# JuliaGenAI/ColBERT.jl

Measured on AMD Instinct MI355X. Metric: queries/sec, top-1000 on 1M-passage corpus, higher is better.
Workload: dtype f32

## Files before the change

### colbert.jl_amd/csrc/approx_kernels.hpp

```cpp
#pragma once
#include <hip/hip_fp16.h>

#include <algorithm>

#include "common.hpp"
#include "search_kernels.hpp"

namespace clb {

typedef __bf16 bf16x8 __attribute__((ext_vector_type(8)));
typedef uint32_t u32x4 __attribute__((ext_vector_type(4)));
typedef uint32_t u32x4_a4 __attribute__((ext_vector_type(4), aligned(4)));
typedef float f32x4_a4 __attribute__((ext_vector_type(4), aligned(4)));

constexpr float kEpsSafety = 1.25f;

inline bool approx_supported(int dim, int nbits) { return dim == kDim && nbits == 2; }
inline size_t approx_cells_bytes(int64_t B, int64_t K, int64_t ) { return (size_t)B * K * 16 * 4 + 2048; }

__device__ __forceinline__ uint32_t f32_to_bf16_rne(float f) {
    const uint32_t u = __float_as_uint(f);
    return (u + 0x7fffu + ((u >> 16) & 1u)) >> 16;
}
__device__ __forceinline__ uint32_t pack_bf16(float lo, float hi) {
// ... 860 lines not shown
    const uint32_t cmask = (1u << cbits) - 1u;
    const int lane = threadIdx.x & 63;
    const int r = lane & 31, h = lane >> 5;
    const int x = blockIdx.x & 7;
    const int wg = blockIdx.x >> 3;
    const int wg_per_group = gridDim.x >> 3;
    const int wave = __builtin_amdgcn_readfirstlane(threadIdx.x >> 6);
    __shared__ __attribute__((aligned(16))) unsigned char lut_s[kApproxLdsLut];
    __shared__ __attribute__((aligned(16))) float invx[kApproxThreads / 64][2 * kStepRows];
    constexpr int kSlotBytes = CELL8 ? 1024 : 2048;
    constexpr int kRingBytes = 3 * kSlotBytes;
    __shared__ __attribute__((aligned(16))) unsigned char ring_s[GL ? (kApproxThreads / 64) * kRingBytes : 16];
    constexpr int kStageBytes = 16 * 64 + 64;
    __shared__ __attribute__((aligned(16))) unsigned char stage_s[ROWS ? 16 : (kApproxThreads / 64) * kStageBytes];
    unsigned char* mystage = stage_s + (ROWS ? 0 : wave * kStageBytes);
    for (int i = threadIdx.x; i < 256 * 32; i += kApproxThreads) {
        const int v = i >> 5;
        *reinterpret_cast<uint2*>(lut_s + (size_t)i * 8) =
            make_uint2(pack_f16(weights[v & 3], weights[(v >> 2) & 3]), pack_f16(weights[(v >> 4) & 3], weights[(v >> 6) & 3]));
    }
    __syncthreads();
    const char* lut = reinterpret_cast<const char*>(lut_s);
    float* myinv = invx[wave];
    const uint32_t lane8 = 8u * (uint32_t)r;
    unsigned char* myring = ring_s + (GL ? wave * kRingBytes : 0);
    const uint32_t ring_lds = (uint32_t)(uintptr_t)(__attribute__((address_space(3))) unsigned char*)myring;
    const uint32_t gl_poff = 16u * (((uint32_t)lane - (((uint32_t)lane >> 4) & 3u)) & 3u);
    const int gl_src0 = (int)((uint32_t)lane & ~3u);
    const int gl_src1 = gl_src0 + 64;
    const uint32_t gl_rot = ((uint32_t)r >> 2) & 3u;
// ... 31 lines not shown
                float4 hi = *reinterpret_cast<const float4*>(qrow + 8 * s + 4);
                if (r >= T) { lo = make_float4(0.f, 0.f, 0.f, 0.f); hi = lo; }
                if (CELL8) {
                    lo.x *= ts.y; lo.y *= ts.y; lo.z *= ts.y; lo.w *= ts.y;
                    hi.x *= ts.y; hi.y *= ts.y; hi.z *= ts.y; hi.w *= ts.y;
                }
                qb[s] = u32x4{pack_f16(lo.x, lo.y), pack_f16(lo.z, lo.w), pack_f16(hi.x, hi.y), pack_f16(hi.z, hi.w)};
            }
        }
        const uint2* hdr = cand_hdr + (size_t)b * cand_cap;
        const char* c16 = reinterpret_cast<const char*>(cells16 + (size_t)b * K * (CELL8 ? 8 : 16));
        const uint32_t h16 = 16u * (uint32_t)h;
        float* out = scores + (size_t)b * cand_cap;
        uint16_t* tmax = tokmax + (size_t)b * cand_cap * 32 + r;
        const int* lst = ROWS ? list + (size_t)b * cand_cap : nullptr;
        unsigned long long* rmask = ROWS ? rowmask + (size_t)b * cand_cap * 4 : nullptr;
        const float window = ROWS ? 2.f * eps_pair[b] : 0.f;
        const int n = ROWS ? nlist[b] : ncand[b];
        const int n_waves = wg_count * (kApproxThreads / 64) * nsub;
        const int my_wave = (sub * wg_count + wg_index) * (kApproxThreads / 64) + wave;
        const int per_wave = (n + n_waves - 1) / n_waves;
        const int j_first = min(n, my_wave * per_wave), j_end = min(n, j_first + per_wave);
        unsigned long long wm0 = 0, wm1 = 0, wm2 = 0, wm3 = 0;

        for (int j0 = j_first; j0 < j_end; j0 += 64) {
        const int jl = j0 + lane;
        int slot_l = jl < j_end ? jl : j0;
        if (ROWS) slot_l = lst[slot_l];
        const uint2 hv = hdr[slot_l];
        const int nd = j_end - j0 < 64 ? j_end - j0 : 64;
        int it_k = 0;
        uint32_t it_off = __builtin_amdgcn_readlane(hv.x, 0);
        int it_len = (int)__builtin_amdgcn_readlane(hv.y, 0);
        int it_slot = __builtin_amdgcn_readlane(slot_l, 0);
        int it_base = 0;

#define CLB_STAGE_A(RB, CV, PM, TAG)                                                                    \
    {                                                                                                       \
// ... 147 lines not shown
         \
        float v[16];                                                                                        \
        _Pragma("unroll") for (int i = 0; i < 16; ++i) { v[i] = ACC[i] * iq[i >> 2][i & 3]; asm volatile("" : "+v"(v[i])); } \
        if (ROWS) {                                                                                         \
            const __half pmh = *reinterpret_cast<const __half*>(&PM);                                       \
            const float lo = r < T ? __half2float(pmh) - window : __builtin_inff();    \
             \
             \
             \
            uint32_t lm = 0;                                                                                \
            _Pragma("unroll") for (int i = 0; i < 16; ++i) lm |= !((CELL8 ? v[i] * stp : v[i]) < lo) ? (1u << i) : 0u; \
            lm |= (uint32_t)__builtin_amdgcn_update_dpp(0, (int)lm, 0xB1, 0xf, 0xf, true);         \
            lm |= (uint32_t)__builtin_amdgcn_update_dpp(0, (int)lm, 0x4E, 0xf, 0xf, true);         \
            lm |= (uint32_t)__builtin_amdgcn_update_dpp(0, (int)lm, 0x141, 0xf, 0xf, true);    \
            lm |= (uint32_t)__builtin_amdgcn_update_dpp(0, (int)lm, 0x140, 0xf, 0xf, true);      \
            const uint32_t m0_ = __builtin_amdgcn_readlane(lm, 0) | __builtin_amdgcn_readlane(lm, 16);      \
            const uint32_t m1_ = __builtin_amdgcn_readlane(lm, 32) | __builtin_amdgcn_readlane(lm, 48);     \
             \
            uint32_t bits = ((m0_ & 0xFu) | ((m0_ & 0xF0u) << 4) | ((m0_ & 0xF00u) << 8) | ((m0_ & 0xF000u) << 12)) | \
                            (((m1_ & 0xFu) | ((m1_ & 0xF0u) << 4) | ((m1_ & 0xF00u) << 8) | ((m1_ & 0xF000u) << 12)) << 4); \
            if (TAG.rows < kStepRows) bits &= (1u << TAG.rows) - 1u;        \
            const unsigned long long wbits = (unsigned long long)bits << (TAG.base & 32);                   \
            const int wi = TAG.base >> 6;                                                                   \
            wm0 |= wi == 0 ? wbits : 0ull;                                                                  \
            wm1 |= wi == 1 ? wbits : 0ull;                                                                  \
            wm2 |= wi == 2 ? wbits : 0ull;                                                                  \
            wm3 |= wi == 3 ? wbits : 0ull;                                                                  \
            if (TAG.last) {                                                                                 \
                if (lane == 0 && TAG.j >= 0) {                                                              \
                    unsigned long long* o = rmask + (size_t)TAG.j * 4;                                      \
                    o[0] = wm0; o[1] = wm1; o[2] = wm2; o[3] = wm3;                                         \
                }                                                                                           \
                wm0 = wm1 = wm2 = wm3 = 0;                                                                  \
            }                                                                                               \
        } else {                                                                                            \
            if (TAG.g) {               \
                const float q0_ = fmaxf(fmaxf(fmaxf(v[0], v[1]), v[2]), v[3]);                              \
                const float q1_ = fmaxf(fmaxf(fmaxf(v[4], v[5]), v[6]), v[7]);                              \
                const float q2_ = fmaxf(fmaxf(fmaxf(v[8], v[9]), v[10]), v[11]);                            \
                const float q3_ = fmaxf(fmaxf(fmaxf(v[12], v[13]), v[14]), v[15]);                          \
                const float mh_ = fmaxf(fmaxf(mx, q0_), fmaxf(TAG.g > 1 ? q1_ : kNegInf, TAG.g > 2 ? q2_ : kNegInf)); \
                CLB_PASSAGE_END(mh_, TAG.jh, 1);                                                            \
                mx = fmaxf(fmaxf(TAG.g > 1 ? kNegInf : q1_, TAG.g > 2 ? kNegInf : q2_), q3_);               \
            } else {                                                                                        \
            float m01 = fmaxf(fmaxf(v[0], v[1]), v[2]);                                                     \
            float m23 = fmaxf(fmaxf(v[3], v[4]), v[5]);                                                     \
            float m45 = fmaxf(fmaxf(v[6], v[7]), v[8]);                                                     \
            float m67 = fmaxf(fmaxf(v[9], v[10]), v[11]);                                                   \
// ... 589 lines not shown
```

### colbert.jl_amd/csrc/search.hip

```cpp
#include <algorithm>
#include <atomic>
#include <cstdlib>
#include <cstring>
#include <memory>
#include <numeric>

#include "append_kernels.hpp"
#include "approx_kernels.hpp"
#include "generic_kernels.hpp"
#include "remove_kernels.hpp"
#include "search_kernels.hpp"
#include "sort.hpp"

using namespace clb;

namespace {

enum KernelId {
    KID_CENTROID_SCORES = 0,
    KID_TOPN,
    KID_MARK,
    KID_COMPACT,
    KID_SCORE_EXACT,
    KID_SCORE_APPROX,
// ... 209 lines not shown
    }
    CLB_TRY(w.cand_hdr.ensure(sizeof(uint2) * B * w.cand_cap));
    CLB_TRY(w.scores.ensure(sizeof(float) * B * w.cand_cap));
    CLB_TRY(w.list.ensure(sizeof(int) * B * w.cand_cap));
    CLB_TRY(w.nlist.ensure(sizeof(int) * B));
    CLB_TRY(w.thresh.ensure(sizeof(float) * B * 2));
    CLB_TRY(w.outp.ensure(sizeof(int64_t) * B * k));
    CLB_TRY(w.outs.ensure(sizeof(float) * B * k));
    CLB_TRY(w.flags.ensure(sizeof(int) * B));
    if (!w.stats.p) {
        CLB_TRY(w.stats.ensure(sizeof(unsigned long long) * 8));
        CLB_HIP(hipMemset(w.stats.p, 0, sizeof(unsigned long long) * 8));
    }
    if (s->approx_ok && Ttuned > 0) {
        CLB_TRY(w.cells_q.ensure(approx_cells_bytes(B, s->K, Tpad)));
        CLB_TRY(w.rowmask.ensure(sizeof(unsigned long long) * 4 * B * w.cand_cap));
        CLB_TRY(w.eps_pair.ensure(sizeof(float) * B));
        CLB_TRY(w.tokmax.ensure(sizeof(uint16_t) * 32 * B * w.cand_cap));
    }
    w.Bcap = B; w.Tcap = T; w.Ttuned = Ttuned; w.npcap = nprobe; w.kcap = k;
    w.filt_cap = std::max(w.filt_cap, filt_count);
    CLB_HIP(hipStreamSynchronize(s->stream));
    return CLB_OK;
}

int ensure_workspace(clb_searcher* s, Workspace& w, int64_t B, int64_t T, int64_t nprobe, int64_t k, size_t filt_count = 0) {
    const int rc = ensure_workspace_sized(s, w, B, T, nprobe, k, filt_count);
    if (rc) {
        w.Bcap = 0;
        if (rc == CLB_ENOMEM && filt_count > w.filt_cap)
            return fail(CLB_EUNSUPPORTED, "no room for the candidate buffers of a filter of %zu passages (CLB_FILTER_ALL, %lld "
// ... 441 lines not shown
        Timed t(s, KID_TOPK, st);
        const int ranked = list != nullptr;
        if (ranked)
            hipLaunchKernelGGL(topk_rank_kernel, dim3(kRankBlocks, B), dim3(1024), 0, st, w.scores.as<float>(),
                               w.cand.as<uint32_t>(), w.ncand.as<int>(), list, nlist, k, w.cand_cap, s->pid_offset,
                               q.d_out_pids, q.d_out_scores, w.flags.as<int>(), q.d_n_cand);
        CLB_TRY(launch_topk(s, w, st, q, 0, B, list, nlist, ranked));
    } else {
        s->prof.chain = nullptr;
        CLB_TRY(launch_topk(s, w, st, q, 0, B, list, nlist, 0));
    }
    if (s->prof.counters) {
        hipLaunchKernelGGL(batch_stats_kernel, dim3(32, B), dim3(256), 0, st, w.cand.as<uint32_t>(),
                           w.ncand.as<int>(), list, nlist, s->doc_off.as<uint32_t>(), w.cand_cap,
                           w.stats.as<unsigned long long>(),
                           subset ? w.rowmask.as<unsigned long long>() : (const unsigned long long*)nullptr);
    }
    CLB_HIP(hipGetLastError());
    return CLB_OK;
}

int check_filters(const clb_searcher* s, const clb_filter* const* filters, int64_t B, int scope, size_t* filt_count) {
    *filt_count = 0;
    if (scope != CLB_FILTER_CANDIDATES && scope != CLB_FILTER_ALL)
        return fail(CLB_EARGUMENT, "scope must be CLB_FILTER_CANDIDATES (0) or CLB_FILTER_ALL (1), got %d", scope);
    if (!filters) return CLB_OK;
    for (int64_t b = 0; b < B; ++b) {
        const clb_filter* f = filters[b];
        if (!f) continue;
        if (f->owner != s->serial)
            return fail(CLB_EARGUMENT, "the filter of query %lld was made for another searcher", (long long)b);
// ... 986 lines not shown
    CLB_TRY(use_device(s->device));
    CLB_HIP(hipDeviceSynchronize());
    unsigned long long h[8] = {0};
    for (auto& w : s->ws) {
        unsigned long long t[8] = {0};
        if (w.stats.p) CLB_HIP(hipMemcpy(t, w.stats.p, sizeof t, hipMemcpyDeviceToHost));
        for (int i = 0; i < 8; ++i) h[i] += t[i];
    }
    if (cand_docs) *cand_docs = (int64_t)h[0];
    if (cand_embs) *cand_embs = (int64_t)h[1];
    if (rescored_docs) *rescored_docs = (int64_t)h[2];
    if (rescored_embs) *rescored_embs = (int64_t)h[3];
    return CLB_OK;
}

}
```

### colbert.jl_amd/csrc/search_kernels.hpp

```cpp
#pragma once
#include <hip/hip_fp16.h>

#include <type_traits>

#include "common.hpp"

namespace clb {

typedef float f32x16 __attribute__((ext_vector_type(16)));
typedef float f32x4 __attribute__((ext_vector_type(4)));

constexpr int kDim = 128;
constexpr int kCentTileStride = 132;
constexpr int kMaxTopK = 16384;

static __global__ __launch_bounds__(128) void centroid_scores_kernel(const float* __restrict__ C,
                                                               const float* __restrict__ Q,
                                                               float* __restrict__ cells, int K, int T,
                                                               int TT, int n_tiles) {
    extern __shared__ __attribute__((aligned(16))) float lds[];
    const int wave = threadIdx.x >> 6, lane = threadIdx.x & 63;
    const int i = lane & 31, h = lane >> 5;
    const int b = blockIdx.y / TT, tt = blockIdx.y % TT;
    const int Tpad = TT * 32;
// ... 654 lines not shown
#pragma unroll
    for (int width = 16; width >= 1; width >>= 1) {
        const int t = __popc(x & ((1u << width) - 1u));
        if (loc >= t) { x >>= width; add += width; loc -= t; }
    }
    return (uint32_t)add;
}

static __global__ __launch_bounds__(256, 3) void score_exact_flat_kernel(
    const float* __restrict__ C, const float* __restrict__ weights, const uint32_t* __restrict__ codes0,
    const uint8_t* __restrict__ residuals, const uint2* __restrict__ cand_hdr, const float* __restrict__ Q,
    float* __restrict__ scores, int T, size_t cand_cap, const int* __restrict__ list,
    const int* __restrict__ nlist, const unsigned long long* __restrict__ rowmask) {
    constexpr int NBITS = 2;
    __shared__ float tbl[weight_table_floats<NBITS>()];
    __shared__ __attribute__((aligned(16))) float qlds[16 * 64 * 4];
    __shared__ __attribute__((aligned(16))) float ctiles[4 * 512 * 4];
    fill_weight_table<NBITS>(tbl, weights);
    const int lane = threadIdx.x & 63;
    const int r = lane & 15, g = lane >> 4;
    const int wave = __builtin_amdgcn_readfirstlane(threadIdx.x >> 6);
    float* ctile = ctiles + wave * 2048;
    const int c4 = lane & 31, rhalf = lane >> 5;
    const float4* qv = reinterpret_cast<const float4*>(qlds) + lane;

#define CLB_REP8(X) X(0) X(1) X(2) X(3) X(4) X(5) X(6) X(7)
#define CLB_ROW_DECL(m) float4 rowA##m;
#define CLB_ROW_LOAD(P, CODE, m)                                                                               \
    {                                                                                                          \
        const uint32_t ca = __builtin_amdgcn_readlane(CODE, 2 * m), cb = __builtin_amdgcn_readlane(CODE, 2 * m + 1); \
        row##P##m = *reinterpret_cast<const float4*>(C + (size_t)(rhalf ? cb : ca) * kDim + 4 * c4);           \
    }
#define CLB_ROW_LOAD8(P, CODE)                                                                                 \
    CLB_ROW_LOAD(P, CODE, 0) CLB_ROW_LOAD(P, CODE, 1) CLB_ROW_LOAD(P, CODE, 2) CLB_ROW_LOAD(P, CODE, 3)        \
    CLB_ROW_LOAD(P, CODE, 4) CLB_ROW_LOAD(P, CODE, 5) CLB_ROW_LOAD(P, CODE, 6) CLB_ROW_LOAD(P, CODE, 7)
#define CLB_ROW_STORE(P, m)                                                                                    \
    {      \
        float* sl_ = ctile + (c4 * 16 + ((2 * m + rhalf) ^ (c4 & 15))) * 4;                                    \
        const int ro_ = 2 * ((((2 * m + rhalf) >> 3) ^ (c4 >> 3)) & 1);                                        \
        *reinterpret_cast<float2*>(sl_ + ro_) = make_float2(row##P##m.x, row##P##m.y);                         \
        *reinterpret_cast<float2*>(sl_ + (ro_ ^ 2)) = make_float2(row##P##m.z, row##P##m.w);                   \
    }
#define CLB_ROW_STORE8(P)                                                                                      \
    CLB_ROW_STORE(P, 0) CLB_ROW_STORE(P, 1) CLB_ROW_STORE(P, 2) CLB_ROW_STORE(P, 3)                            \
    CLB_ROW_STORE(P, 4) CLB_ROW_STORE(P, 5) CLB_ROW_STORE(P, 6) CLB_ROW_STORE(P, 7)

    {
        const int b = blockIdx.y;
        __syncthreads();
        for (int i = threadIdx.x; i < 16 * 64; i += 256) {
            const int k = i >> 6, l = i & 63;
            const int rr = l & 15, gg = l >> 4;
            const int t0 = rr, t1 = rr + 16;
            const float* qa = Q + ((size_t)b * T + (t0 < T ? t0 : T - 1)) * kDim + gg;
            const float* qb = Q + ((size_t)b * T + (t1 < T ? t1 : T - 1)) * kDim + gg;
            float4 v;
            v.x = t0 < T ? qa[8 * k] : 0.f;
            v.y = t1 < T ? qb[8 * k] : 0.f;
            v.z = t0 < T ? qa[8 * k + 4] : 0.f;
            v.w = t1 < T ? qb[8 * k + 4] : 0.f;
            *reinterpret_cast<float4*>(qlds + (size_t)i * 4) = v;
        }
        __syncthreads();
        const int n = nlist[b];
        const int* lst = list + (size_t)b * cand_cap;
        const uint2* hdr = cand_hdr + (size_t)b * cand_cap;
        const unsigned long long* mw = rowmask + (size_t)b * cand_cap * 4;
        float* out = scores + (size_t)b * cand_cap;
        const int stride = gridDim.x * 4;

        for (int j0 = blockIdx.x * 4 + wave; j0 < n; j0 += 64 * stride) {
            const int jl = j0 + lane * stride;
            const int jj = jl < n ? jl : j0;
            const int slot_l = lst[jj];
            const uint2 hv = hdr[slot_l];
            const unsigned long long mk0 = mw[(size_t)jj * 4], mk1 = mw[(size_t)jj * 4 + 1],
                                     mk2 = mw[(size_t)jj * 4 + 2], mk3 = mw[(size_t)jj * 4 + 3];
            const bool ident_l = (int)hv.y > kMaxMaskedRows;
            const uint32_t nj_l = ident_l ? (hv.y | 0x80000000u)
                                          : (uint32_t)(__popcll(mk0) + __popcll(mk1) + __popcll(mk2) + __popcll(mk3));
            const int nd = (n - j0 + stride - 1) / stride < 64 ? (n - j0 + stride - 1) / stride : 64;
            int it_k = 0, it_base = 0;
            uint32_t it_off, it_nj;
            int it_slot;
            unsigned long long it_m0, it_m1, it_m2, it_m3;
#define CLB_IT_LOAD(KK)                                                                                        \
    {                                                                                                          \
        it_off = __builtin_amdgcn_readlane(hv.x, KK);                                                          \
        it_nj = __builtin_amdgcn_readlane(nj_l, KK);                                                           \
        it_slot = __builtin_amdgcn_readlane(slot_l, KK);                                                       \
        it_m0 = ((unsigned long long)(uint32_t)__builtin_amdgcn_readlane((uint32_t)(mk0 >> 32), KK) << 32) | (uint32_t)__builtin_amdgcn_readlane((uint32_t)mk0, KK); \
        it_m1 = ((unsigned long long)(uint32_t)__builtin_amdgcn_readlane((uint32_t)(mk1 >> 32), KK) << 32) | (uint32_t)__builtin_amdgcn_readlane((uint32_t)mk1, KK); \
        it_m2 = ((unsigned long long)(uint32_t)__builtin_amdgcn_readlane((uint32_t)(mk2 >> 32), KK) << 32) | (uint32_t)__builtin_amdgcn_readlane((uint32_t)mk2, KK); \
        it_m3 = ((unsigned long long)(uint32_t)__builtin_amdgcn_readlane((uint32_t)(mk3 >> 32), KK) << 32) | (uint32_t)__builtin_amdgcn_readlane((uint32_t)mk3, KK); \
    }
            CLB_IT_LOAD(0)

#define CLB_XSTAGE_A(CODE, R0, R1, TAG)                                                                        \
    {                                                                                                          \
        const bool live = it_k < nd;                                                                           \
        const int nj = (int)(it_nj & 0x7fffffffu);                                                             \
        const int rem = nj - it_base;                                                                          \
        uint32_t e;                                                                                            \
        if (rem < 16 && it_k + 1 < nd) {                  \
            const int kn = it_k + 1;                                                                           \
            const uint32_t nx_off = __builtin_amdgcn_readlane(hv.x, kn);                                       \
            const uint32_t nx_nj = __builtin_amdgcn_readlane(nj_l, kn);                                        \
            const int nx_slot = __builtin_amdgcn_readlane(slot_l, kn);                                         \
            const unsigned long long nx_m0 = ((unsigned long long)(uint32_t)__builtin_amdgcn_readlane((uint32_t)(mk0 >> 32), kn) << 32) | (uint32_t)__builtin_amdgcn_readlane((uint32_t)mk0, kn); \
            const unsigned long long nx_m1 = ((unsigned long long)(uint32_t)__builtin_amdgcn_readlane((uint32_t)(mk1 >> 32), kn) << 32) | (uint32_t)__builtin_amdgcn_readlane((uint32_t)mk1, kn); \
            const unsigned long long nx_m2 = ((unsigned long long)(uint32_t)__builtin_amdgcn_readlane((uint32_t)(mk2 >> 32), kn) << 32) | (uint32_t)__builtin_amdgcn_readlane((uint32_t)mk2, kn); \
            const unsigned long long nx_m3 = ((unsigned long long)(uint32_t)__builtin_amdgcn_readlane((uint32_t)(mk3 >> 32), kn) << 32) | (uint32_t)__builtin_amdgcn_readlane((uint32_t)mk3, kn); \
            const int njn = (int)(nx_nj & 0x7fffffffu);                                                        \
            const int take = 16 - rem < njn ? 16 - rem : njn;                                                  \
            const bool second = r >= rem;                  \
            const int ia = it_base + r;                                                                        \
            const int ib = r - rem < njn ? r - rem : njn - 1;                                                  \
            const int idx = second ? ib : ia;                                                                  \
            const bool ident = ((second ? nx_nj : it_nj) & 0x80000000u) != 0u;                                 \
            const uint32_t row = ident ? (uint32_t)idx                                                         \
                                       : nth_set_bit_256(second ? nx_m0 : it_m0, second ? nx_m1 : it_m1,       \
                                                         second ? nx_m2 : it_m2, second ? nx_m3 : it_m3, idx); \
            e = (second ? nx_off : it_off) + row;                                                              \
            const int last1 = njn <= 16 - rem;                                                                 \
            TAG.slot = it_slot;                                                                                \
            TAG.slot1 = nx_slot;                                                                               \
            TAG.info = rem | 0x100 | (last1 << 9);                                                             \
            it_k += 1;                                                                                         \
            if (last1) {                                                                                       \
                it_k += 1;                                                                                     \
                const int kk = it_k < 64 ? it_k : 63;                                                          \
                CLB_IT_LOAD(kk)                                                                                \
                it_base = 0;                                                                                   \
            } else {                                                                                           \
                it_off = nx_off; it_nj = nx_nj; it_slot = nx_slot;                                             \
                it_m0 = nx_m0; it_m1 = nx_m1; it_m2 = nx_m2; it_m3 = nx_m3;                                    \
                it_base = take;                                                                                \
            }                                                                                                  \
        } else {                                                                                               \
            const int idx = it_base + r < nj ? it_base + r : nj - 1;                                           \
            const uint32_t row = (it_nj & 0x80000000u) ? (uint32_t)idx : nth_set_bit_256(it_m0, it_m1, it_m2, it_m3, idx); \
            e = live ? it_off + row : 0u;                                                                      \
            const int last = it_base + 16 >= nj;                                                               \
            TAG.slot = live ? it_slot : -1;                                                                    \
            TAG.slot1 = -1;                                                                                    \
            TAG.info = 16 | (last << 8);                                                                       \
            it_base += 16;                                                                                     \
            if (last) {                                                                                        \
                it_k += 1;                                                                                     \
                const int kk = it_k < 64 ? it_k : 63;                                                          \
                CLB_IT_LOAD(kk)                                                                                \
                it_base = 0;                                                                                   \
            }                                                                                                  \
        }                                                                                                      \
        CODE = codes0[e];                                                                                      \
        const uint4* rp = reinterpret_cast<const uint4*>(residuals + (size_t)e * 32);                          \
        R0 = rp[0];                                                                                            \
        R1 = rp[1];                                                                                            \
    }
#define CLB_XSTAGE_C(P, R0, R1, TAG, CODE_NEXT2)                                                               \
    {                                                                                                          \
        CLB_ROW_STORE8(P)                                                                                      \
        __builtin_amdgcn_wave_barrier();                                                                       \
        const uint32_t R[8] = {R0.x, R0.y, R0.z, R0.w, R1.x, R1.y, R1.z, R1.w};                                \
        float x[32];                                                                                           \
        decompress_lane_dims_fast<NBITS>(nullptr, R, g, tbl, x, ctile, r);                                     \
        __builtin_amdgcn_wave_barrier();                                                                       \
        CLB_ROW_LOAD8(P, CODE_NEXT2)                                                                           \
        f32x4 a0 = {0.f, 0.f, 0.f, 0.f}, a1 = {0.f, 0.f, 0.f, 0.f};                                            \
        float4 qnext = qv[0];                                                                                  \
        _Pragma("unroll") for (int k = 0; k < 16; ++k) {                                                       \
            const float4 q = qnext;                                                                            \
            if (k < 15) qnext = qv[(k + 1) * 64];                                                              \
            a0 = __builtin_amdgcn_mfma_f32_16x16x4f32(x[2 * k], q.x, a0, 0, 0, 0);                             \
            a1 = __builtin_amdgcn_mfma_f32_16x16x4f32(x[2 * k], q.y, a1, 0, 0, 0);                             \
            a0 = __builtin_amdgcn_mfma_f32_16x16x4f32(x[2 * k + 1], q.z, a0, 0, 0, 0);                         \
            a1 = __builtin_amdgcn_mfma_f32_16x16x4f32(x[2 * k + 1], q.w, a1, 0, 0, 0);                         \
        }                                                                                                      \
         \
         \
        float c0, c1, n0 = kNegInf, n1 = kNegInf;                                                              \
        const int p_ = TAG.info & 31;                                                                          \
        if (p_ >= 16) {                                                                                        \
            c0 = fmaxf(fmaxf(m0, fmaxf(a0[0], a0[1])), fmaxf(a0[2], a0[3]));                                   \
            c1 = fmaxf(fmaxf(m1, fmaxf(a1[0], a1[1])), fmaxf(a1[2], a1[3]));                                   \
        } else {                                                                                               \
            c0 = m0;                                                                                           \
            c1 = m1;                                                                                           \
            _Pragma("unroll") for (int q_ = 0; q_ < 4; ++q_) {                                                 \
                const bool first_ = 4 * g + q_ < p_;                                                           \
                c0 = fmaxf(c0, first_ ? a0[q_] : kNegInf);                                                     \
                c1 = fmaxf(c1, first_ ? a1[q_] : kNegInf);                                                     \
                n0 = fmaxf(n0, first_ ? kNegInf : a0[q_]);                                                     \
                n1 = fmaxf(n1, first_ ? kNegInf : a1[q_]);                                                     \
            }                                                                                                  \
        }                                                                                                      \
        {                                                                                                      \
            const int nfin_ = ((TAG.info >> 8) & 1) + ((TAG.info >> 9) & 1);        \
            int cs_ = TAG.slot;                                                                                \
            _Pragma("unroll 1") for (int f_ = 0; f_ < nfin_; ++f_) {                                           \
                c0 = fmaxf(c0, __shfl_xor(c0, 16, 64));                                                        \
                c0 = fmaxf(c0, __shfl_xor(c0, 32, 64));                                                        \
                c1 = fmaxf(c1, __shfl_xor(c1, 16, 64));                                                        \
                c1 = fmaxf(c1, __shfl_xor(c1, 32, 64));                                                        \
                 \
                 \
                 \
                float total = 0.f;                                                                             \
                _Pragma("unroll") for (int t = 0; t < 32; ++t) {                                               \
                    const uint32_t sv = __builtin_amdgcn_readlane(__float_as_uint(t < 16 ? c0 : c1), t & 15);  \
                    total = total + __uint_as_float(t < T ? sv : 0u);                                          \
                }                                                                                              \
                if (lane == 0 && cs_ >= 0) out[cs_] = total;                                                   \
                c0 = n0;                                                                                       \
                c1 = n1;                                                                                       \
                n0 = kNegInf;                                                                                  \
                n1 = kNegInf;                                                                                  \
                cs_ = TAG.slot1;                                                                               \
            }                                                                                                  \
        }                                                                                                      \
        m0 = c0;                                                                                               \
        m1 = c1;                                                                                               \
    }

            float m0 = kNegInf, m1 = kNegInf;
            uint32_t cd0, cd1, cd2;
            uint4 ra0, rb0, ra1, rb1, ra2, rb2;
            ExactStepTag t0, t1, t2;
            CLB_REP8(CLB_ROW_DECL)
            CLB_XSTAGE_A(cd0, ra0, rb0, t0)
            CLB_XSTAGE_A(cd1, ra1, rb1, t1)
            CLB_ROW_LOAD8(A, cd0)
            while (t0.slot >= 0) {
                CLB_XSTAGE_A(cd2, ra2, rb2, t2)
                CLB_XSTAGE_C(A, ra0, rb0, t0, cd1)
                CLB_XSTAGE_A(cd0, ra0, rb0, t0)
                CLB_XSTAGE_C(A, ra1, rb1, t1, cd2)
                CLB_XSTAGE_A(cd1, ra1, rb1, t1)
                CLB_XSTAGE_C(A, ra2, rb2, t2, cd0)
            }
#undef CLB_IT_LOAD
#undef CLB_XSTAGE_A
#undef CLB_XSTAGE_C
        }
    }
#undef CLB_REP8
#undef CLB_ROW_DECL
#undef CLB_ROW_LOAD
#undef CLB_ROW_LOAD8
#undef CLB_ROW_STORE
#undef CLB_ROW_STORE8
}

__device__ __forceinline__ void radix_pick(const int* hist, int rem, uint32_t prefix, int shift,
                                           uint32_t* s_prefix, int* s_remaining) {
    const int lane = threadIdx.x & 63;
// ... 351 lines not shown
    dst[i] = src[(size_t)perm[e] * pieces + q];
}

static __global__ void codes_to_zero_based_kernel(uint32_t* __restrict__ codes, int64_t n, uint32_t K,
                                           int* __restrict__ err) {
    const int64_t i = (int64_t)blockIdx.x * blockDim.x + threadIdx.x;
    if (i >= n) return;
    const uint32_t c = codes[i];
    if (c < 1u || c > K) { atomicOr(err, 2); codes[i] = 0; } else codes[i] = c - 1u;
}

static __global__ void batch_stats_kernel(const uint32_t* __restrict__ cand, const int* __restrict__ ncand,
                                   const int* __restrict__ list, const int* __restrict__ nlist,
                                   const uint32_t* __restrict__ doc_off, size_t cand_cap,
                                   unsigned long long* __restrict__ stats,
                                   const unsigned long long* __restrict__ rowmask ) {
    const int b = blockIdx.y;
    const uint32_t* cnd = cand + (size_t)b * cand_cap;
    unsigned long long embs = 0, lembs = 0;
    const int n = ncand[b];
    for (int i = blockIdx.x * blockDim.x + threadIdx.x; i < n; i += gridDim.x * blockDim.x) {
        const uint32_t p = cnd[i];
        embs += doc_off[p + 1] - doc_off[p];
    }
    const int nl = list ? nlist[b] : 0;
    for (int i = blockIdx.x * blockDim.x + threadIdx.x; i < nl; i += gridDim.x * blockDim.x) {
        const uint32_t p = cnd[list[(size_t)b * cand_cap + i]];
        const uint32_t len = doc_off[p + 1] - doc_off[p];
        if (rowmask && len <= (uint32_t)kMaxMaskedRows) {
            const unsigned long long* mw = rowmask + ((size_t)b * cand_cap + i) * 4;
            lembs += __popcll(mw[0]) + __popcll(mw[1]) + __popcll(mw[2]) + __popcll(mw[3]);
        } else {
            lembs += len;
        }
    }
    for (int o = 32; o > 0; o >>= 1) {
        embs += __shfl_down(embs, o, 64);
        lembs += __shfl_down(lembs, o, 64);
    }
    if ((threadIdx.x & 63) == 0) {
        if (embs) atomicAdd(&stats[1], embs);
        if (lembs) atomicAdd(&stats[3], lembs);
    }
    if (blockIdx.x == 0 && threadIdx.x == 0) {
        atomicAdd(&stats[0], (unsigned long long)n);
        atomicAdd(&stats[2], (unsigned long long)nl);
    }
}

__device__ __forceinline__ bool rec_before(float s, int64_t p, float s2, int64_t p2) {
    return s > s2 || (s == s2 && p < p2);
}
static __global__ __launch_bounds__(256) void merge_topk_kernel(const int64_t* __restrict__ pids,
                                                         const float* __restrict__ scores, int k, int n_lists,
                                                         int B, size_t pid_stride, size_t score_stride,
                                                         int64_t* __restrict__ out_pids,
                                                         float* __restrict__ out_scores) {
// ... 33 lines not shown
```

### colbert.jl_amd/searcher.py

```python
from __future__ import annotations

import ctypes as C
import os
from typing import Optional

import numpy as np

from . import storage
from ._lib import BoundsError, ColBERTError, check, colmajor, fptr, i64, lib
from .config import ColBERTConfig


_SCOPES = {"candidates": 0, "all": 1}


def _scope_code(scope) -> int:
    if scope not in _SCOPES:
        raise ColBERTError(f"scope must be 'candidates' or 'all', got {scope!r}")
    return _SCOPES[scope]


class PassageFilter:

    def __init__(self, searcher: "Searcher", handle, count: int):
# ... 322 lines not shown
    def profile_enable(self, on: bool = True, counters: bool = False):
        check(lib().clb_profile_enable(self._h, C.c_int((2 if counters else 1) if on else 0)))

    def profile_read(self) -> dict:
        cap = 16
        names = (C.c_char_p * cap)(); ms = (C.c_double * cap)(); cnt = (C.c_int64 * cap)()
        n = lib().clb_profile_read(self._h, names, ms, cnt, cap)
        if n < 0:
            check(10)
        return {names[i].decode(): {"ms": ms[i], "launches": cnt[i]} for i in range(n)}

    def last_batch_stats(self) -> dict:
        a, b, c, d = i64(0), i64(0), i64(0), i64(0)
        check(lib().clb_last_batch_stats(self._h, C.byref(a), C.byref(b), C.byref(c), C.byref(d)))
        return {"cand_docs": a.value, "cand_embs": b.value, "rescored_docs": c.value, "rescored_embs": d.value}


class TextSearch:

    def __init__(self, searcher: Searcher, k: int, nprobe: Optional[int] = None, graph: bool = True):
        import torch
        from .distributed import DeviceSearch
        if searcher.encoder is None or searcher.encoder.tokenizer is None:
            raise ColBERTError("text search needs an encoder with a tokenizer attached to the Searcher")
        self.s, self.enc, self.k = searcher, searcher.encoder, int(k)
        cfg = self.enc.config
        self.T = int(cfg.query_maxlen)
        self.dev = torch.device("cuda", searcher.device)
        tok = self.enc.tokenizer
        self.h_ids = torch.empty((1, self.T), dtype=torch.int32).pin_memory()
# ... 157 lines not shown
```

### include/colbert_hip.h

```cpp
#ifndef COLBERT_HIP_H
#define COLBERT_HIP_H
#include <stdint.h>
#ifdef __cplusplus
extern "C" {
#endif

#define CLB_OK 0
#define CLB_EDIMENSION 1
#define CLB_EDOMAIN 2
#define CLB_EBOUNDS 3
#define CLB_EARGUMENT 4
#define CLB_EHIP 10
#define CLB_EUNSUPPORTED 11
#define CLB_ENOMEM 12

typedef struct clb_searcher clb_searcher;

const char* clb_version(void);
const char* clb_last_error(void);
int clb_device_count(void);
int clb_measure_copy_rate(int device, int64_t bytes, int reps, double* gb_per_s);
int clb_measure_read_rate(int device, int64_t bytes, int reps, double* gb_per_s);

int clb_searcher_create(int device, int64_t dim, int nbits, int64_t K,
// ... 70 lines not shown
int clb_debug_scores(clb_searcher* s, const float* Q, int64_t T, int64_t nprobe, int64_t k, int64_t cap,
                     int64_t* out_pids, float* out_approx, float* out_exact, int64_t* n_out, float* tau,
                     float* eps, int64_t* n_rescore);

int clb_merge_topk_device(int device, const int64_t* d_pids, const float* d_scores, int64_t k,
                          int64_t n_lists, int64_t B, int64_t* d_out_pids, float* d_out_scores,
                          void* hip_stream);
int64_t clb_packed_topk_bytes(int64_t k, int64_t B);
int clb_merge_topk_packed_device(int device, const void* d_packed, int64_t k, int64_t n_lists, int64_t B,
                                 int64_t* d_out_pids, float* d_out_scores, void* hip_stream);

int clb_profile_enable(clb_searcher* s, int on);
int clb_profile_read(clb_searcher* s, const char** names, double* total_ms, int64_t* launches, int cap);
int clb_last_batch_stats(clb_searcher* s, int64_t* cand_docs, int64_t* cand_embs, int64_t* rescored_docs,
                         int64_t* rescored_embs);

int clb_decompress(int device, int64_t dim, int nbits, const float* centroids, int64_t K,
                   const float* bucket_weights, int64_t n_weights, const uint32_t* codes, int64_t n_codes,
                   const uint8_t* residuals, int64_t res_rows, int64_t res_cols, float* out);
int clb_maxsim(int device, const float* Q, int64_t dim, int64_t T, const float* D, int64_t n_D,
               const int64_t* pids, int64_t n_pids, const int64_t* doclens, int64_t n_docs, float* scores);
int clb_compress_into_codes(int device, uint32_t* codes, int64_t n_codes, const float* centroids,
                            int64_t dim, int64_t K, const float* embs, int64_t n);
int clb_compress(int device, const float* centroids, int64_t K, const float* bucket_cutoffs,
                 int64_t n_cutoffs, int64_t dim, int nbits, const float* embs, int64_t n,
                 uint32_t* codes, uint8_t* residuals);
int clb_normalize_columns(int device, float* X, int64_t dim, int64_t n);

int clb_kmeans(int device, const float* data, int64_t dim, int64_t n, float* centroids, int64_t K,
               int64_t max_iters, float tol, int64_t point_bsize, int32_t* assignments,
// ... 109 lines not shown
```

Baseline: 28850.

## Split exact rescoring row masks by query-token half to skip unneeded rows

The approximate kernel now writes a separate row mask for each 16-token half of the query, using per-wave LDS accumulation instead of register bitmasks, which doubles the rowmask storage. The exact rescoring kernel handles 32 candidates per pass and walks each candidate twice, once per token half, using only that half's mask. The low-half partial sum is parked in a register and added when the high half finishes. The goal is to skip decoding document rows that can only matter for one half of the query tokens. The cost is an extra pass, more mask traffic, and new stats counters plus an API for per-half row counts.

```diff
diff --git a/colbert.jl_amd/csrc/approx_kernels.hpp b/colbert.jl_amd/csrc/approx_kernels.hpp
--- a/colbert.jl_amd/csrc/approx_kernels.hpp
+++ b/colbert.jl_amd/csrc/approx_kernels.hpp
@@ -898,6 +898,9 @@
     constexpr int kStageBytes = 16 * 64 + 64;
     __shared__ __attribute__((aligned(16))) unsigned char stage_s[ROWS ? 16 : (kApproxThreads / 64) * kStageBytes];
     unsigned char* mystage = stage_s + (ROWS ? 0 : wave * kStageBytes);
+    __shared__ uint32_t mask_s[ROWS ? (kApproxThreads / 64) * 32 : 1];
+    uint32_t* mymask = mask_s + (ROWS ? wave * 32 : 0);
+    if (ROWS && threadIdx.x < (kApproxThreads / 64) * 32) mask_s[threadIdx.x] = 0u;
     for (int i = threadIdx.x; i < 256 * 32; i += kApproxThreads) {
         const int v = i >> 5;
         *reinterpret_cast<uint2*>(lut_s + (size_t)i * 8) =
@@ -959,14 +962,13 @@
         float* out = scores + (size_t)b * cand_cap;
         uint16_t* tmax = tokmax + (size_t)b * cand_cap * 32 + r;
         const int* lst = ROWS ? list + (size_t)b * cand_cap : nullptr;
-        unsigned long long* rmask = ROWS ? rowmask + (size_t)b * cand_cap * 4 : nullptr;
+        unsigned long long* rmask = ROWS ? rowmask + (size_t)b * cand_cap * 8 : nullptr;
         const float window = ROWS ? 2.f * eps_pair[b] : 0.f;
         const int n = ROWS ? nlist[b] : ncand[b];
         const int n_waves = wg_count * (kApproxThreads / 64) * nsub;
         const int my_wave = (sub * wg_count + wg_index) * (kApproxThreads / 64) + wave;
         const int per_wave = (n + n_waves - 1) / n_waves;
         const int j_first = min(n, my_wave * per_wave), j_end = min(n, j_first + per_wave);
-        unsigned long long wm0 = 0, wm1 = 0, wm2 = 0, wm3 = 0;
 
         for (int j0 = j_first; j0 < j_end; j0 += 64) {
         const int jl = j0 + lane;
@@ -1144,24 +1146,31 @@
             lm |= (uint32_t)__builtin_amdgcn_update_dpp(0, (int)lm, 0x4E, 0xf, 0xf, true);         \
             lm |= (uint32_t)__builtin_amdgcn_update_dpp(0, (int)lm, 0x141, 0xf, 0xf, true);    \
             lm |= (uint32_t)__builtin_amdgcn_update_dpp(0, (int)lm, 0x140, 0xf, 0xf, true);      \
-            const uint32_t m0_ = __builtin_amdgcn_readlane(lm, 0) | __builtin_amdgcn_readlane(lm, 16);      \
-            const uint32_t m1_ = __builtin_amdgcn_readlane(lm, 32) | __builtin_amdgcn_readlane(lm, 48);     \
              \
-            uint32_t bits = ((m0_ & 0xFu) | ((m0_ & 0xF0u) << 4) | ((m0_ & 0xF00u) << 8) | ((m0_ & 0xF000u) << 12)) | \
-                            (((m1_ & 0xFu) | ((m1_ & 0xF0u) << 4) | ((m1_ & 0xF00u) << 8) | ((m1_ & 0xF000u) << 12)) << 4); \
-            if (TAG.rows < kStepRows) bits &= (1u << TAG.rows) - 1u;        \
-            const unsigned long long wbits = (unsigned long long)bits << (TAG.base & 32);                   \
-            const int wi = TAG.base >> 6;                                                                   \
-            wm0 |= wi == 0 ? wbits : 0ull;                                                                  \
-            wm1 |= wi == 1 ? wbits : 0ull;                                                                  \
-            wm2 |= wi == 2 ? wbits : 0ull;                                                                  \
-            wm3 |= wi == 3 ? wbits : 0ull;                                                                  \
+             \
+             \
+             \
+            uint32_t sp_ = ((lm & 0xFu) | ((lm & 0xF0u) << 4) | ((lm & 0xF00u) << 8) | ((lm & 0xF000u) << 12)) << (4 * h); \
+            sp_ &= TAG.rows < kStepRows ? (1u << TAG.rows) - 1u : 0xffffffffu;                              \
+             \
+             \
+             \
+             \
+             \
+            const int wd_ = TAG.base >> 5;                                                                  \
+            int ln_ = lane;                                                                                 \
+            asm volatile("" : "+v"(ln_));      \
+            if ((ln_ & 15) == 0 && wd_ < 8 && TAG.j >= 0) mymask[wd_ + 8 * (((ln_ >> 3) & 2) | (ln_ >> 5))] = sp_; \
             if (TAG.last) {                                                                                 \
-                if (lane == 0 && TAG.j >= 0) {                                                              \
-                    unsigned long long* o = rmask + (size_t)TAG.j * 4;                                      \
-                    o[0] = wm0; o[1] = wm1; o[2] = wm2; o[3] = wm3;                                         \
+                __builtin_amdgcn_wave_barrier();                                                            \
+                if (ln_ < 16) {          \
+                    const int d_ = (ln_ & 7) + 16 * (ln_ >> 3);                                             \
+                    const uint32_t mv_ = mymask[d_] | mymask[d_ + 8];                                       \
+                    if (TAG.j >= 0) reinterpret_cast<uint32_t*>(rmask + (size_t)TAG.j * 8)[ln_] = mv_;      \
+                    mymask[d_] = 0u;                                                                        \
+                    mymask[d_ + 8] = 0u;                                                                    \
                 }                                                                                           \
-                wm0 = wm1 = wm2 = wm3 = 0;                                                                  \
+                __builtin_amdgcn_wave_barrier();                                                            \
             }                                                                                               \
         } else {                                                                                            \
             if (TAG.g) {               \
diff --git a/colbert.jl_amd/csrc/search.hip b/colbert.jl_amd/csrc/search.hip
--- a/colbert.jl_amd/csrc/search.hip
+++ b/colbert.jl_amd/csrc/search.hip
@@ -247,7 +247,7 @@
     }
     if (s->approx_ok && Ttuned > 0) {
         CLB_TRY(w.cells_q.ensure(approx_cells_bytes(B, s->K, Tpad)));
-        CLB_TRY(w.rowmask.ensure(sizeof(unsigned long long) * 4 * B * w.cand_cap));
+        CLB_TRY(w.rowmask.ensure(sizeof(unsigned long long) * 8 * B * w.cand_cap));
         CLB_TRY(w.eps_pair.ensure(sizeof(float) * B));
         CLB_TRY(w.tokmax.ensure(sizeof(uint16_t) * 32 * B * w.cand_cap));
     }
@@ -719,7 +719,7 @@
         hipLaunchKernelGGL(batch_stats_kernel, dim3(32, B), dim3(256), 0, st, w.cand.as<uint32_t>(),
                            w.ncand.as<int>(), list, nlist, s->doc_off.as<uint32_t>(), w.cand_cap,
                            w.stats.as<unsigned long long>(),
-                           subset ? w.rowmask.as<unsigned long long>() : (const unsigned long long*)nullptr);
+                           subset ? w.rowmask.as<unsigned long long>() : (const unsigned long long*)nullptr, T);
     }
     CLB_HIP(hipGetLastError());
     return CLB_OK;
@@ -1736,4 +1736,20 @@
     return CLB_OK;
 }
 
-}
+int clb_last_batch_half_rows(clb_searcher* s, int64_t* rows_lo, int64_t* rows_hi) {
+    if (!s) return fail(CLB_EARGUMENT, "null searcher");
+    CLB_TRY(use_device(s->device));
+    CLB_HIP(hipDeviceSynchronize());
+    unsigned long long h[2] = {0, 0};
+    for (auto& w : s->ws) {
+        unsigned long long t[8] = {0};
+        if (w.stats.p) CLB_HIP(hipMemcpy(t, w.stats.p, sizeof t, hipMemcpyDeviceToHost));
+        h[0] += t[4];
+        h[1] += t[5];
+    }
+    if (rows_lo) *rows_lo = (int64_t)h[0];
+    if (rows_hi) *rows_hi = (int64_t)h[1];
+    return CLB_OK;
+}
+
+}
diff --git a/colbert.jl_amd/csrc/search_kernels.hpp b/colbert.jl_amd/csrc/search_kernels.hpp
--- a/colbert.jl_amd/csrc/search_kernels.hpp
+++ b/colbert.jl_amd/csrc/search_kernels.hpp
@@ -692,7 +692,7 @@
     const int* __restrict__ nlist, const unsigned long long* __restrict__ rowmask) {
     constexpr int NBITS = 2;
     __shared__ float tbl[weight_table_floats<NBITS>()];
-    __shared__ __attribute__((aligned(16))) float qlds[16 * 64 * 4];
+    __shared__ __attribute__((aligned(16))) float qlds[2 * 16 * 64 * 2];
     __shared__ __attribute__((aligned(16))) float ctiles[4 * 512 * 4];
     fill_weight_table<NBITS>(tbl, weights);
     const int lane = threadIdx.x & 63;
@@ -700,7 +700,8 @@
     const int wave = __builtin_amdgcn_readfirstlane(threadIdx.x >> 6);
     float* ctile = ctiles + wave * 2048;
     const int c4 = lane & 31, rhalf = lane >> 5;
-    const float4* qv = reinterpret_cast<const float4*>(qlds) + lane;
+    const float2* qv = reinterpret_cast<const float2*>(qlds) + lane;
+    const bool has_hi = T > 16;
 
 #define CLB_REP8(X) X(0) X(1) X(2) X(3) X(4) X(5) X(6) X(7)
 #define CLB_ROW_DECL(m) float4 rowA##m;
@@ -726,42 +727,41 @@
     {
         const int b = blockIdx.y;
         __syncthreads();
-        for (int i = threadIdx.x; i < 16 * 64; i += 256) {
-            const int k = i >> 6, l = i & 63;
+        for (int i = threadIdx.x; i < 2 * 16 * 64; i += 256) {
+            const int hf = i >> 10, k = (i >> 6) & 15, l = i & 63;
             const int rr = l & 15, gg = l >> 4;
-            const int t0 = rr, t1 = rr + 16;
-            const float* qa = Q + ((size_t)b * T + (t0 < T ? t0 : T - 1)) * kDim + gg;
-            const float* qb = Q + ((size_t)b * T + (t1 < T ? t1 : T - 1)) * kDim + gg;
-            float4 v;
-            v.x = t0 < T ? qa[8 * k] : 0.f;
-            v.y = t1 < T ? qb[8 * k] : 0.f;
-            v.z = t0 < T ? qa[8 * k + 4] : 0.f;
-            v.w = t1 < T ? qb[8 * k + 4] : 0.f;
-            *reinterpret_cast<float4*>(qlds + (size_t)i * 4) = v;
+            const int t = 16 * hf + rr;
+            const float* qa = Q + ((size_t)b * T + (t < T ? t : T - 1)) * kDim + gg;
+            float2 v;
+            v.x = t < T ? qa[8 * k] : 0.f;
+            v.y = t < T ? qa[8 * k + 4] : 0.f;
+            *reinterpret_cast<float2*>(qlds + (size_t)i * 2) = v;
         }
         __syncthreads();
         const int n = nlist[b];
         const int* lst = list + (size_t)b * cand_cap;
         const uint2* hdr = cand_hdr + (size_t)b * cand_cap;
-        const unsigned long long* mw = rowmask + (size_t)b * cand_cap * 4;
+        const unsigned long long* mw = rowmask + (size_t)b * cand_cap * 8;
         float* out = scores + (size_t)b * cand_cap;
         const int stride = gridDim.x * 4;
 
-        for (int j0 = blockIdx.x * 4 + wave; j0 < n; j0 += 64 * stride) {
-            const int jl = j0 + lane * stride;
+        for (int j0 = blockIdx.x * 4 + wave; j0 < n; j0 += 32 * stride) {
+            const int jl = j0 + (lane & 31) * stride;
             const int jj = jl < n ? jl : j0;
+            const int mh_ = 4 * (lane >> 5);
             const int slot_l = lst[jj];
             const uint2 hv = hdr[slot_l];
-            const unsigned long long mk0 = mw[(size_t)jj * 4], mk1 = mw[(size_t)jj * 4 + 1],
-                                     mk2 = mw[(size_t)jj * 4 + 2], mk3 = mw[(size_t)jj * 4 + 3];
             const bool ident_l = (int)hv.y > kMaxMaskedRows;
+            const unsigned long long mk0 = mw[(size_t)jj * 8 + mh_], mk1 = mw[(size_t)jj * 8 + mh_ + 1],
+                                     mk2 = mw[(size_t)jj * 8 + mh_ + 2], mk3 = mw[(size_t)jj * 8 + mh_ + 3];
             const uint32_t nj_l = ident_l ? (hv.y | 0x80000000u)
-                                          : (uint32_t)(__popcll(mk0) + __popcll(mk1) + __popcll(mk2) + __popcll(mk3));
-            const int nd = (n - j0 + stride - 1) / stride < 64 ? (n - j0 + stride - 1) / stride : 64;
-            int it_k = 0, it_base = 0;
+                                    : (uint32_t)(__popcll(mk0) + __popcll(mk1) + __popcll(mk2) + __popcll(mk3));
+            const int nd = (n - j0 + stride - 1) / stride < 32 ? (n - j0 + stride - 1) / stride : 32;
+            int it_k = 0, it_base = 0, it_half = 0;
             uint32_t it_off, it_nj;
             int it_slot;
             unsigned long long it_m0, it_m1, it_m2, it_m3;
+            float park = 0.f;
 #define CLB_IT_LOAD(KK)                                                                                        \
     {                                                                                                          \
         it_off = __builtin_amdgcn_readlane(hv.x, KK);                                                          \
@@ -773,15 +773,27 @@
         it_m3 = ((unsigned long long)(uint32_t)__builtin_amdgcn_readlane((uint32_t)(mk3 >> 32), KK) << 32) | (uint32_t)__builtin_amdgcn_readlane((uint32_t)mk3, KK); \
     }
             CLB_IT_LOAD(0)
+#define CLB_IT_NEXT                                                                                            \
+    {                                                                                                          \
+        it_k += 1;                                                                                             \
+        if (it_k >= nd && it_half == 0 && has_hi) {                                                            \
+            it_half = 1;                                                                                       \
+            it_k = 0;                                                                                          \
+        }                                                                                                      \
+        const int kk = (it_k < 32 ? it_k : 31) + 32 * it_half;                                                 \
+        CLB_IT_LOAD(kk)                                                                                        \
+        it_base = 0;                                                                                           \
+    }
 
 #define CLB_XSTAGE_A(CODE, R0, R1, TAG)                                                                        \
     {                                                                                                          \
         const bool live = it_k < nd;                                                                           \
         const int nj = (int)(it_nj & 0x7fffffffu);                                                             \
         const int rem = nj - it_base;                                                                          \
+        const int hk_ = (it_half << 10) | (it_k << 16);                                                        \
         uint32_t e;                                                                                            \
         if (rem < 16 && it_k + 1 < nd) {                  \
-            const int kn = it_k + 1;                                                                           \
+            const int kn = it_k + 1 + 32 * it_half;                                                            \
             const uint32_t nx_off = __builtin_amdgcn_readlane(hv.x, kn);                                       \
             const uint32_t nx_nj = __builtin_amdgcn_readlane(nj_l, kn);                                        \
             const int nx_slot = __builtin_amdgcn_readlane(slot_l, kn);                                         \
@@ -803,13 +815,10 @@
             const int last1 = njn <= 16 - rem;                                                                 \
             TAG.slot = it_slot;                                                                                \
             TAG.slot1 = nx_slot;                                                                               \
-            TAG.info = rem | 0x100 | (last1 << 9);                                                             \
+            TAG.info = rem | 0x100 | (last1 << 9) | hk_ | ((it_k + 1) << 24);                                  \
             it_k += 1;                                                                                         \
             if (last1) {                                                                                       \
-                it_k += 1;                                                                                     \
-                const int kk = it_k < 64 ? it_k : 63;                                                          \
-                CLB_IT_LOAD(kk)                                                                                \
-                it_base = 0;                                                                                   \
+                CLB_IT_NEXT                                                                                    \
             } else {                                                                                           \
                 it_off = nx_off; it_nj = nx_nj; it_slot = nx_slot;                                             \
                 it_m0 = nx_m0; it_m1 = nx_m1; it_m2 = nx_m2; it_m3 = nx_m3;                                    \
@@ -822,14 +831,9 @@
             const int last = it_base + 16 >= nj;                                                               \
             TAG.slot = live ? it_slot : -1;                                                                    \
             TAG.slot1 = -1;                                                                                    \
-            TAG.info = 16 | (last << 8);                                                                       \
+            TAG.info = 16 | (last << 8) | hk_;                                                                 \
             it_base += 16;                                                                                     \
-            if (last) {                                                                                        \
-                it_k += 1;                                                                                     \
-                const int kk = it_k < 64 ? it_k : 63;                                                          \
-                CLB_IT_LOAD(kk)                                                                                \
-                it_base = 0;                                                                                   \
-            }                                                                                                  \
+            if (last) CLB_IT_NEXT                                                                              \
         }                                                                                                      \
         CODE = codes0[e];                                                                                      \
         const uint4* rp = reinterpret_cast<const uint4*>(residuals + (size_t)e * 32);                          \
@@ -845,63 +849,60 @@
         decompress_lane_dims_fast<NBITS>(nullptr, R, g, tbl, x, ctile, r);                                     \
         __builtin_amdgcn_wave_barrier();                                                                       \
         CLB_ROW_LOAD8(P, CODE_NEXT2)                                                                           \
-        f32x4 a0 = {0.f, 0.f, 0.f, 0.f}, a1 = {0.f, 0.f, 0.f, 0.f};                                            \
-        float4 qnext = qv[0];                                                                                  \
+        const int half_ = (TAG.info >> 10) & 1;                                                                \
+        const float2* qh_ = qv + half_ * (16 * 64);                     \
+        f32x4 a0 = {0.f, 0.f, 0.f, 0.f};                                                                       \
+        float2 qnext = qh_[0];                                                                                 \
         _Pragma("unroll") for (int k = 0; k < 16; ++k) {                                                       \
-            const float4 q = qnext;                                                                            \
-            if (k < 15) qnext = qv[(k + 1) * 64];                                                              \
+            const float2 q = qnext;                                                                            \
+            if (k < 15) qnext = qh_[(k + 1) * 64];                                                             \
             a0 = __builtin_amdgcn_mfma_f32_16x16x4f32(x[2 * k], q.x, a0, 0, 0, 0);                             \
-            a1 = __builtin_amdgcn_mfma_f32_16x16x4f32(x[2 * k], q.y, a1, 0, 0, 0);                             \
-            a0 = __builtin_amdgcn_mfma_f32_16x16x4f32(x[2 * k + 1], q.z, a0, 0, 0, 0);                         \
-            a1 = __builtin_amdgcn_mfma_f32_16x16x4f32(x[2 * k + 1], q.w, a1, 0, 0, 0);                         \
+            a0 = __builtin_amdgcn_mfma_f32_16x16x4f32(x[2 * k + 1], q.y, a0, 0, 0, 0);                         \
         }                                                                                                      \
          \
          \
-        float c0, c1, n0 = kNegInf, n1 = kNegInf;                                                              \
+        float c0, n0 = kNegInf;                                                                                \
         const int p_ = TAG.info & 31;                                                                          \
         if (p_ >= 16) {                                                                                        \
             c0 = fmaxf(fmaxf(m0, fmaxf(a0[0], a0[1])), fmaxf(a0[2], a0[3]));                                   \
-            c1 = fmaxf(fmaxf(m1, fmaxf(a1[0], a1[1])), fmaxf(a1[2], a1[3]));                                   \
         } else {                                                                                               \
             c0 = m0;                                                                                           \
-            c1 = m1;                                                                                           \
             _Pragma("unroll") for (int q_ = 0; q_ < 4; ++q_) {                                                 \
                 const bool first_ = 4 * g + q_ < p_;                                                           \
                 c0 = fmaxf(c0, first_ ? a0[q_] : kNegInf);                                                     \
-                c1 = fmaxf(c1, first_ ? a1[q_] : kNegInf);                                                     \
                 n0 = fmaxf(n0, first_ ? kNegInf : a0[q_]);                                                     \
-                n1 = fmaxf(n1, first_ ? kNegInf : a1[q_]);                                                     \
             }                                                                                                  \
         }                                                                                                      \
         {                                                                                                      \
             const int nfin_ = ((TAG.info >> 8) & 1) + ((TAG.info >> 9) & 1);        \
             int cs_ = TAG.slot;                                                                                \
+            int ck_ = (TAG.info >> 16) & 127;                                                                  \
             _Pragma("unroll 1") for (int f_ = 0; f_ < nfin_; ++f_) {                                           \
                 c0 = fmaxf(c0, __shfl_xor(c0, 16, 64));                                                        \
                 c0 = fmaxf(c0, __shfl_xor(c0, 32, 64));                                                        \
-                c1 = fmaxf(c1, __shfl_xor(c1, 16, 64));                                                        \
-                c1 = fmaxf(c1, __shfl_xor(c1, 32, 64));                                                        \
                  \
                  \
                  \
-                float total = 0.f;                                                                             \
-                _Pragma("unroll") for (int t = 0; t < 32; ++t) {                                               \
-                    const uint32_t sv = __builtin_amdgcn_readlane(__float_as_uint(t < 16 ? c0 : c1), t & 15);  \
-                    total = total + __uint_as_float(t < T ? sv : 0u);                                          \
+                float total = half_ ? __uint_as_float(__builtin_amdgcn_readlane(__float_as_uint(park), ck_ & 63)) : 0.f; \
+                _Pragma("unroll") for (int t = 0; t < 16; ++t) {                                               \
+                    const uint32_t sv = __builtin_amdgcn_readlane(__float_as_uint(c0), t);                     \
+                    total = total + __uint_as_float(16 * half_ + t < T ? sv : 0u);                             \
                 }                                                                                              \
-                if (lane == 0 && cs_ >= 0) out[cs_] = total;                                                   \
+                if (half_ || !has_hi) {                                                                        \
+                    if (lane == 0 && cs_ >= 0) out[cs_] = total;                                               \
+                } else if (cs_ >= 0) {                                                                         \
+                    park = lane == ck_ ? total : park;                                                         \
+                }                                                                                              \
                 c0 = n0;                                                                                       \
-                c1 = n1;                                                                                       \
                 n0 = kNegInf;                                                                                  \
-                n1 = kNegInf;                                                                                  \
                 cs_ = TAG.slot1;                                                                               \
+                ck_ = (TAG.info >> 24) & 127;                                                                  \
             }                                                                                                  \
         }                                                                                                      \
         m0 = c0;                                                                                               \
-        m1 = c1;                                                                                               \
-    }
-
-            float m0 = kNegInf, m1 = kNegInf;
+    }
+
+            float m0 = kNegInf;
             uint32_t cd0, cd1, cd2;
             uint4 ra0, rb0, ra1, rb1, ra2, rb2;
             ExactStepTag t0, t1, t2;
@@ -918,6 +919,7 @@
                 CLB_XSTAGE_C(A, ra2, rb2, t2, cd0)
             }
 #undef CLB_IT_LOAD
+#undef CLB_IT_NEXT
 #undef CLB_XSTAGE_A
 #undef CLB_XSTAGE_C
         }
@@ -1299,10 +1301,10 @@
                                    const int* __restrict__ list, const int* __restrict__ nlist,
                                    const uint32_t* __restrict__ doc_off, size_t cand_cap,
                                    unsigned long long* __restrict__ stats,
-                                   const unsigned long long* __restrict__ rowmask ) {
+                                   const unsigned long long* __restrict__ rowmask , int T) {
     const int b = blockIdx.y;
     const uint32_t* cnd = cand + (size_t)b * cand_cap;
-    unsigned long long embs = 0, lembs = 0;
+    unsigned long long embs = 0, lembs = 0, lo_rows = 0, hi_rows = 0;
     const int n = ncand[b];
     for (int i = blockIdx.x * blockDim.x + threadIdx.x; i < n; i += gridDim.x * blockDim.x) {
         const uint32_t p = cnd[i];
@@ -1313,19 +1315,29 @@
         const uint32_t p = cnd[list[(size_t)b * cand_cap + i]];
         const uint32_t len = doc_off[p + 1] - doc_off[p];
         if (rowmask && len <= (uint32_t)kMaxMaskedRows) {
-            const unsigned long long* mw = rowmask + ((size_t)b * cand_cap + i) * 4;
-            lembs += __popcll(mw[0]) + __popcll(mw[1]) + __popcll(mw[2]) + __popcll(mw[3]);
+            const unsigned long long* mw = rowmask + ((size_t)b * cand_cap + i) * 8;
+            lembs += __popcll(mw[0] | mw[4]) + __popcll(mw[1] | mw[5]) + __popcll(mw[2] | mw[6]) + __popcll(mw[3] | mw[7]);
+            lo_rows += __popcll(mw[0]) + __popcll(mw[1]) + __popcll(mw[2]) + __popcll(mw[3]);
+            hi_rows += __popcll(mw[4]) + __popcll(mw[5]) + __popcll(mw[6]) + __popcll(mw[7]);
         } else {
             lembs += len;
+            if (rowmask) {
+                lo_rows += len;
+                hi_rows += T > 16 ? len : 0u;
+            }
         }
     }
     for (int o = 32; o > 0; o >>= 1) {
         embs += __shfl_down(embs, o, 64);
         lembs += __shfl_down(lembs, o, 64);
+        lo_rows += __shfl_down(lo_rows, o, 64);
+        hi_rows += __shfl_down(hi_rows, o, 64);
     }
     if ((threadIdx.x & 63) == 0) {
         if (embs) atomicAdd(&stats[1], embs);
         if (lembs) atomicAdd(&stats[3], lembs);
+        if (lo_rows) atomicAdd(&stats[4], lo_rows);
+        if (hi_rows) atomicAdd(&stats[5], hi_rows);
     }
     if (blockIdx.x == 0 && threadIdx.x == 0) {
         atomicAdd(&stats[0], (unsigned long long)n);
diff --git a/colbert.jl_amd/searcher.py b/colbert.jl_amd/searcher.py
--- a/colbert.jl_amd/searcher.py
+++ b/colbert.jl_amd/searcher.py
@@ -360,6 +360,11 @@
         a, b, c, d = i64(0), i64(0), i64(0), i64(0)
         check(lib().clb_last_batch_stats(self._h, C.byref(a), C.byref(b), C.byref(c), C.byref(d)))
         return {"cand_docs": a.value, "cand_embs": b.value, "rescored_docs": c.value, "rescored_embs": d.value}
+
+    def last_batch_half_rows(self) -> dict:
+        a, b = i64(0), i64(0)
+        check(lib().clb_last_batch_half_rows(self._h, C.byref(a), C.byref(b)))
+        return {"rows_lo": a.value, "rows_hi": b.value}
 
 
 class TextSearch:
diff --git a/include/colbert_hip.h b/include/colbert_hip.h
--- a/include/colbert_hip.h
+++ b/include/colbert_hip.h
@@ -108,6 +108,7 @@
 int clb_profile_read(clb_searcher* s, const char** names, double* total_ms, int64_t* launches, int cap);
 int clb_last_batch_stats(clb_searcher* s, int64_t* cand_docs, int64_t* cand_embs, int64_t* rescored_docs,
                          int64_t* rescored_embs);
+int clb_last_batch_half_rows(clb_searcher* s, int64_t* rows_lo, int64_t* rows_hi);
 
 int clb_decompress(int device, int64_t dim, int nbits, const float* centroids, int64_t K,
                    const float* bucket_weights, int64_t n_weights, const uint32_t* codes, int64_t n_codes,
```

After: 29170, median of 6. 1.01x the previous value.
